# febrianrachmadi/dep-gan-im

Measured on AMD Instinct MI355X. Metric: 2D slices/sec (G+2D+GP train step), 256x256x1 fp32, higher is better.
Workload: dtype f32; 1 GPU; DEP-GAN-IM twoCritics canonical train step (critic-Y2 + critic-DEM + G update, WGAN-GP), batch 32 per GPU, 256x256x1; per_gpu_batch=32, global_batch=32, parallelism=dp1

## Files before the change

### dep_gan_im_amd/csrc/common.h

```cpp
#pragma once
#include <hip/hip_runtime.h>
#include <stdint.h>
#include <stddef.h>

typedef float f32x2 __attribute__((ext_vector_type(2)));
typedef float f32x4 __attribute__((ext_vector_type(4)));
typedef float f32x16 __attribute__((ext_vector_type(16)));

struct TView {
  float* p;
  long sB, sY, sX;
};

static inline TView make_view(float* p, int H, int W, int C) {
  TView v;
  v.p = p;
  v.sX = C;
  v.sY = (long)W * C;
  v.sB = (long)H * W * C;
  return v;
}
static inline TView make_view_slice(float* p, int H, int W, int Ctot, int c0) {
  TView v = make_view(p, H, W, Ctot);
  v.p = p + c0;
// ... 130 lines not shown
  static int cus[DG_MAX_DEVICES] = {};
  const int d = dg_device_slot();
  if (d >= 0 && cus[d]) return cus[d];
  int n = 256;
  hipDeviceProp_t p;
  if (d >= 0 && hipGetDeviceProperties(&p, d) == hipSuccess && p.multiProcessorCount > 0) n = p.multiProcessorCount;
  if (d >= 0) cus[d] = n;
  return n;
}

struct ConvPlan {
  int KS, Cin, Cout;
  int MF;
  int NT;
  int CK;
  int nNT, nCC;
  size_t packedFloats;
  int variant;
  int bf16;
};
ConvPlan dg_plan_conv(int KS, int Cin, int Cout);
ConvPlan dg_plan_conv_items(int KS, int Cin, int Cout, long items);
ConvPlan dg_plan_conv_bf16(int KS, int Cin, int Cout);
ConvPlan dg_plan_conv_split(int KS, int Cin, int Cout, int planes);
int dg_conv_igemm_bf16(const ConvPlan& pl, const ConvArgs& a, hipStream_t st);
static inline size_t dg_plan_elem_bytes(const ConvPlan& pl) { return pl.variant >= 200 ? 2 * (size_t)pl.bf16 : (pl.bf16 ? 2 : 4); }

struct PackJob {
  const float* src;
  float* dst;
  const float* kscale;
  int ntaps, srcI, srcO, io, transpose, flip;
  int NT, CK, nCC, Kdim, Ndim;
  int bf16;
  int tapg;
  int wino;
  unsigned total;
  unsigned per_nt;
  unsigned nt_stride;
  unsigned blk0, nblk;
};
int dg_pack_job(const ConvPlan& pl, const float* src, int srcI, int srcO, int io, int transpose, int flip,
                const float* kscale, float* dst, size_t nt_stride, PackJob* job);
unsigned dg_pack_layout(PackJob* jobs_host, int njobs);
int dg_pack_weights_batch(const PackJob* jobs_dev, int njobs, unsigned nblocks, hipStream_t st);

int dg_pack_weights(const ConvPlan& pl, const float* src, int srcI, int srcO, int io, int transpose, int flip,
                    const float* kscale, float* dst, hipStream_t st);

int dg_conv_igemm(const ConvPlan& pl, const ConvArgs& a, hipStream_t st);
int dg_conv_igemm_check(const ConvPlan& pl, const ConvArgs& a);
bool dg_conv_igemm_wp_supported(const ConvPlan& pl, const ConvArgs& a, bool force);
int dg_conv_igemm_wp(const ConvPlan& pl, const ConvArgs& a, hipStream_t st);
int dg_conv_igemm_tile(const ConvPlan& pl, const ConvArgs& a, hipStream_t st);
bool dg_conv_igemm_head_supported(const ConvPlan& pl, const ConvArgs& a);
ConvPlan dg_plan_conv_wino(int Cin, int Cout);
bool dg_conv_wino_supported(const ConvPlan& pl, const ConvArgs& a);
const char* dg_conv_wino_name(const ConvArgs& a);
int dg_conv_wino(const ConvPlan& pl, const ConvArgs& a, hipStream_t st);
void dg_conv_igemm_name(const ConvPlan& pl, const ConvArgs& a, char* buf, size_t cap);
int dg_conv_direct(int KS, const ConvArgs& a, hipStream_t st);

size_t dg_wgrad_part_floats(int KS, int B, int H, int W, int Cin, int Cout);
int dg_wgrad(int KS, const WgradArgs& a, int* nchunks, hipStream_t st);
int dg_wgrad_finish(const float* part, int nchunks, int ntaps, int Cin, int Cout, const float* scale, float* out,
                    float* raw, int accumulate, int oi, const float* colpart, int colC, const float* colscale,
                    float* colout, float* colraw, hipStream_t st);
int dg_wgrad_finish_rows(const float* part, int nchunks, int ntaps, int Cin, int Cout, const float* scale, float* out,
                         float* raw, int accumulate, int oi, const float* colpart, int colrows, int colC,
                         const float* colscale, float* colout, float* colraw, hipStream_t st);
int dg_wgrad_reduce(const float* part, int nchunks, int ntaps, int Cin, int Cout, const float* scale, float* out,
                    float* raw, int accumulate, int oi, hipStream_t st);

bool dg_wgrad_bf16_supported(int KS, int Cin, int Cout);
size_t dg_wgrad_bf16_part_floats(int KS, int B, int H, int W, int Cin, int Cout);
int dg_wgrad_bf16(int KS, const WgradArgs& a, int* nchunks, hipStream_t st);

size_t dg_wgrad_small_part_floats(int KS, int B, int H, int W, int Cin, int Cout);
int dg_wgrad_small(int KS, const WgradArgs& a, int* nchunks, hipStream_t st);
```

### dep_gan_im_amd/csrc/igemm_conv.hip

```cpp
#include <stdlib.h>

#include "common.h"
#include "epilogue.h"

__device__ __forceinline__ void store_packed(float* dst, size_t i, float v, int bf16) {
  if (bf16) reinterpret_cast<__bf16*>(dst)[i] = (__bf16)v;
  else dst[i] = v;
}
__device__ __forceinline__ void store_split(float* dst, size_t nt_base, int cc, int tap, int n, int k, float v, int planes,
                                            int tapg, int ntaps, int NT, int CK) {
  const int ng = ntaps / tapg, tg = tap / tapg, tl = tap - tg * tapg;
  __bf16* d = reinterpret_cast<__bf16*>(dst) + nt_base + ((size_t)cc * ng + tg) * (size_t)(planes * tapg * NT * CK);
  float rem = v;
  for (int p = 0; p < planes; ++p) {
    const __bf16 hb = (__bf16)rem;
    d[((size_t)p * tapg + tl) * (NT * CK) + (size_t)n * CK + k] = hb;
    rem -= (float)hb;
  }
}

template <int MF>
struct Mfma;
template <>
struct Mfma<32> {
// ... 388 lines not shown
      static DgOncePerDevice once_h;
      if (once_h.need()) {
        HIPCHECK(hipFuncSetAttribute(reinterpret_cast<const void*>(&igemm_conv_head_kernel<false>),
                                     hipFuncAttributeMaxDynamicSharedMemorySize, (int)lds));
        HIPCHECK(hipFuncSetAttribute(reinterpret_cast<const void*>(&igemm_conv_head_kernel<true>),
                                     hipFuncAttributeMaxDynamicSharedMemorySize, (int)lds));
      }
      if (G < total) hipLaunchKernelGGL((igemm_conv_head_kernel<true>), dim3((unsigned)G), dim3(256), lds, st, b);
      else hipLaunchKernelGGL((igemm_conv_head_kernel<false>), dim3((unsigned)G), dim3(256), lds, st, b);
      HIPCHECK(hipGetLastError());
      return DG_OK;
    }
  }
  static DgOncePerDevice once;
  if (once.need()) {
    HIPCHECK(hipFuncSetAttribute(reinterpret_cast<const void*>(&igemm_conv_kernel<MF, KS, CK, TAPG, false>),
                                 hipFuncAttributeMaxDynamicSharedMemorySize, (int)lds));
    HIPCHECK(hipFuncSetAttribute(reinterpret_cast<const void*>(&igemm_conv_kernel<MF, KS, CK, TAPG, true>),
                                 hipFuncAttributeMaxDynamicSharedMemorySize, (int)lds));
  }
  if (G < total)
    hipLaunchKernelGGL((igemm_conv_kernel<MF, KS, CK, TAPG, true>), dim3((unsigned)G), dim3(256), lds, st, b);
  else
    hipLaunchKernelGGL((igemm_conv_kernel<MF, KS, CK, TAPG, false>), dim3((unsigned)G), dim3(256), lds, st, b);
  HIPCHECK(hipGetLastError());
  return DG_OK;
}

static int dispatch_variant(const ConvPlan& pl, const ConvArgs& a, hipStream_t st, char* name_out, size_t name_cap) {
  switch (pl.variant) {
    case 0: return launch_variant<32, 3, 16, 9>(a, st, name_out, name_cap);
    case 1: return launch_variant<16, 3, 16, 9>(a, st, name_out, name_cap);
    case 2: return launch_variant<32, 5, 8, 25>(a, st, name_out, name_cap);
    case 3: return launch_variant<16, 5, 16, 25>(a, st, name_out, name_cap);
    case 4: return launch_variant<32, 1, 32, 1>(a, st, name_out, name_cap);
    case 5: return launch_variant<16, 1, 16, 1>(a, st, name_out, name_cap);
    case 8: return launch_variant<32, 3, 8, 9>(a, st, name_out, name_cap);
  }
  dg_set_error("dg_conv_igemm: bad variant %d", pl.variant);
  return DG_ERR_ARG;
}

bool dg_conv_igemm_head_supported(const ConvPlan& pl, const ConvArgs& a) {
  return (pl.variant == 8 || pl.variant == 9) && !pl.bf16 && a.Cout == 32 && a.groups <= 1 && a.ep.pool.p == nullptr && a.cpt <= 0 &&
         !a.ep.accumulate;
}

void dg_conv_igemm_name(const ConvPlan& pl, const ConvArgs& a, char* buf, size_t cap) {
  if (cap) buf[0] = 0;
  if (pl.variant < 0) { snprintf(buf, cap, "conv_direct"); return; }
  if (pl.bf16) { snprintf(buf, cap, pl.variant >= 200 ? "igemm_split_kernel" : "igemm_bf16_kernel"); return; }
  if (pl.variant == 9) { snprintf(buf, cap, "%s", dg_conv_wino_name(a)); return; }
  if (dg_conv_igemm_wp_supported(pl, a, false)) { snprintf(buf, cap, "igemm_wp_kernel<0>"); return; }
  dispatch_variant(pl, a, nullptr, buf, cap);
}

int dg_conv_igemm_check(const ConvPlan& pl, const ConvArgs& a) {
  if (pl.variant < 0) {
    dg_set_error("dg_conv_igemm: no MFMA variant for KS=%d Cin=%d Cout=%d", pl.KS, pl.Cin, pl.Cout);
    return DG_ERR_UNSUPPORTED;
  }
  auto misaligned = [](const TView& v) {
    return v.p && ((v.sX % 4) || (v.sY % 4) || (v.sB % 4) || (((uintptr_t)v.p) & 15));
  };
  if (misaligned(a.in) || misaligned(a.out) || misaligned(a.ep.res) || misaligned(a.ep.mask) ||
      misaligned(a.ep.out_pre) || (a.Cout % 4) || (a.ep.film_mul && (a.ep.film_ld % 4))) {
    dg_set_error("dg_conv_igemm: views must be 16-byte aligned (pointers, strides and Cout multiples of 4 floats)");
    return DG_ERR_ARG;
  }
  if (a.ep.pool.p && ((a.H | a.W) & 1 || misaligned(a.ep.pool) || a.groups > 1)) {
    dg_set_error("dg_conv_igemm: fused max-pool needs even H, W and a 16-byte aligned pooled view");
    return DG_ERR_ARG;
  }
  if (a.cpt > 0) {
    const int run = a.cpt * pl.CK;
    bool bad = a.groups > 1 || (a.Cin % run) != 0 || a.Cin / run > 4;
    for (int r = 0; !bad && r < a.Cin / run; ++r) bad = (a.in_run_off[r] % 4) != 0;
    if (bad) {
      dg_set_error("dg_conv_igemm: gathered K needs Cin = runs (<= 4) x cpt x %d channels and 16-byte run offsets", pl.CK);
      return DG_ERR_ARG;
    }
  }
  if (a.ep.head_out && !dg_conv_igemm_head_supported(pl, a)) {
    dg_set_error("dg_conv_igemm: the fused head needs the fp32 8-channel-chunk 3x3 kernel, 32 output channels, no pool");
    return DG_ERR_ARG;
  }
  return DG_OK;
}

static int conv_igemm_impl(const ConvPlan& pl, const ConvArgs& a_in, hipStream_t st, bool allow_wp) {
  ConvArgs a = a_in;
  const bool is_bf16 = pl.bf16 != 0;
  DGCHECK(dg_conv_igemm_check(pl, a));
  if (is_bf16) return dg_conv_igemm_bf16(pl, a, st);
  if (pl.variant == 9) return dg_conv_wino(pl, a, st);
  if (allow_wp && dg_conv_igemm_wp_supported(pl, a, false)) return dg_conv_igemm_wp(pl, a, st);
  return dispatch_variant(pl, a, st, nullptr, 0);
}

int dg_conv_igemm(const ConvPlan& pl, const ConvArgs& a, hipStream_t st) { return conv_igemm_impl(pl, a, st, true); }
int dg_conv_igemm_tile(const ConvPlan& pl, const ConvArgs& a, hipStream_t st) { return conv_igemm_impl(pl, a, st, false); }

__global__ void pack_weights_kernel(const float* __restrict__ src, float* __restrict__ dst, int ntaps, int srcI,
                                    int srcO, int io, int transpose, int flip, const float* __restrict__ kscale,
                                    int NT, int CK, int nCC, int Kdim, int Ndim, size_t total, int bf16, int tapg) {
  for (size_t i = blockIdx.x * (size_t)blockDim.x + threadIdx.x; i < total; i += (size_t)gridDim.x * blockDim.x) {
    size_t q = i;
    const int k = (int)(q % CK);
    q /= CK;
    const int n = (int)(q % NT);
    q /= NT;
    const int tap = (int)(q % ntaps);
    q /= ntaps;
    const int cc = (int)(q % nCC);
    const int nt = (int)(q / nCC);
    const int kk = cc * CK + k, nn = nt * NT + n;
    float v = 0.f;
    if (kk < Kdim && nn < Ndim) {
      const int ci = transpose ? nn : kk;
      const int co = transpose ? kk : nn;
      const int ts = flip ? (ntaps - 1 - tap) : tap;
      const size_t off = (size_t)ts * srcI * srcO + (io ? ((size_t)co * srcI + ci) : ((size_t)ci * srcO + co));
      v = src[off];
      if (kscale) v *= kscale[kk];
    }
    if (bf16 >= 2) store_split(dst, (size_t)nt * nCC * ntaps * NT * CK * bf16, cc, tap, n, k, v, bf16, tapg, ntaps, NT, CK);
    else store_packed(dst, i, v, bf16);
  }
}

__global__ __launch_bounds__(256) void pack_weights_batch_kernel(const PackJob* __restrict__ jobs, int njobs) {
  int lo = 0, hi = njobs - 1;
  while (lo < hi) {
    const int mid = (lo + hi + 1) >> 1;
    if (jobs[mid].blk0 <= blockIdx.x) lo = mid; else hi = mid - 1;
  }
  const PackJob J = jobs[lo];
  const unsigned b = blockIdx.x - J.blk0;
  if (J.wino) {
    const unsigned cols = J.total / 16u, plane = (unsigned)(J.NT * J.CK);
    for (unsigned i = b * 256u + threadIdx.x; i < cols; i += J.nblk * 256u) {
      unsigned q = i;
      const int k = (int)(q % J.CK);
      q /= J.CK;
      const int n = (int)(q % J.NT);
      q /= J.NT;
      const int cc = (int)(q % J.nCC);
      const int nt = (int)(q / J.nCC);
      const int kk = cc * J.CK + k, nn = nt * J.NT + n;
// ... 131 lines not shown
```

### dep_gan_im_amd/csrc/igemm_wp.hip

```cpp
#include <stdlib.h>

#include "common.h"
#include "epilogue.h"

namespace {

constexpr int WP_NW = 16;
constexpr int WP_TWX = 18, WP_TWY = 6;
constexpr int WP_PIX = WP_TWX * WP_TWY;
constexpr int WP_CK = 8, WP_CKP = 12;
constexpr int WP_WAVE_FLOATS = WP_PIX * WP_CKP;
constexpr int WP_SLOTS = WP_PIX * 2;
constexpr int WP_PIECES = (WP_SLOTS + 63) / 64;

template <int ABL>
__global__ __launch_bounds__(WP_NW * 64, 1) void igemm_wp_kernel(const ConvArgs a) {
  constexpr int MF = 32, NT = 32, MT = 2, KS = 3, TW = WP_TWX;
  typedef f32x16 acc_t;
  extern __shared__ __attribute__((aligned(16))) float smem[];
  const int tid = threadIdx.x;
  const int lane = tid & 63, wv = tid >> 6;
  const int r = lane & 31, h = lane >> 5;
  const int nCC = a.Cin / WP_CK;
  const int panelFloats = nCC * 9 * NT * WP_CK;
  float* panel = smem;
  float* wbuf = smem + panelFloats + wv * WP_WAVE_FLOATS;

  const unsigned nNT = (unsigned)a.lgy, nSup = (unsigned)a.lgx;
  const int supX = (a.W + 63) >> 6, supY = (a.H + 15) >> 4;
  unsigned id = blockIdx.x;
  auto decode = [&](unsigned i, int& st, int& nt) {
    if ((nSup & 7u) == 0) {
      const unsigned x = i & 7u, sl = i >> 3;
      nt = (int)(sl % nNT);
      st = (int)(x * (nSup >> 3) + sl / nNT);
    } else {
      st = (int)(i % nSup);
      nt = (int)(i / nSup);
    }
  };
  int st0, ntile;
  decode(id, st0, ntile);
  const int n0 = ntile * NT;

  {
    const float* src = a.w + (size_t)ntile * panelFloats;
    const int nq = panelFloats / 4;
    for (int q = tid; q < nq; q += WP_NW * 64) {
      const int row = q >> 1, half = q & 1;
      const f32x4 v = *reinterpret_cast<const f32x4*>(src + (size_t)q * 4);
      *reinterpret_cast<f32x4*>(panel + row * 8 + 4 * (half ^ ((row >> 2) & 1))) = v;
    }
  }
  __syncthreads();

  unsigned xgb[WP_PIECES], xlb[WP_PIECES];
  int xyx[WP_PIECES];
#pragma unroll
  for (int i = 0; i < WP_PIECES; ++i) {
    const int q = min(lane + 64 * i, WP_SLOTS - 1);
    const int pix = q >> 1, part = q & 1;
    const int ly = pix / TW, lx = pix - ly * TW;
    xgb[i] = 4u * (unsigned)(ly * (int)a.in.sY + lx * (int)a.in.sX + part * 4);
    xlb[i] = 4u * (unsigned)(pix * WP_CKP + part * 4);
    xyx[i] = (ly << 16) | (lx << 8) | (part * 4);
  }
  const bool in_last = lane < (WP_SLOTS - 64 * (WP_PIECES - 1));
  const unsigned wb0 = (unsigned)(size_t)(__attribute__((address_space(3))) float*)wbuf;
  int apix[MT];
#pragma unroll
  for (int mt = 0; mt < MT; ++mt) apix[mt] = ((2 * mt + (r >> 4)) * TW + (r & 15)) * WP_CKP + 4 * h;
  const int boff = r * 8 + 4 * (h ^ ((r >> 2) & 1));
  const int wrow = wv & 3, wcol = wv >> 2;

  for (;;) {
    int st, nt_unused;
    decode(id, st, nt_unused);
    const int sx = st % supX;
    int t = st / supX;
    const int sy = t % supY;
    const int b = t / supY;
    const int ty0 = sy * 16 + 4 * wrow, tx0 = sx * 64 + 16 * wcol;
    if (ty0 < a.H && tx0 < a.W) {
      const float* inb = a.in.p + (long)b * a.in.sB;
      const bool interior = ty0 >= 1 && ty0 + 5 <= a.H && tx0 >= 1 && tx0 + 17 <= a.W;
      const char* halo0 = reinterpret_cast<const char*>(inb + ((long)(ty0 - 1) * a.in.sY + (long)(tx0 - 1) * a.in.sX));
      f32x4 xr[WP_PIECES];
      auto prefetch = [&](int cc) {
        const char* src = halo0 + 4 * (long)cc * WP_CK;
        if (interior) {
#pragma unroll
          for (int i = 0; i < WP_PIECES - 1; ++i) xr[i] = *reinterpret_cast<const f32x4*>(src + xgb[i]);
          if (in_last) xr[WP_PIECES - 1] = *reinterpret_cast<const f32x4*>(src + xgb[WP_PIECES - 1]);
        } else {
#pragma unroll
          for (int i = 0; i < WP_PIECES; ++i) {
            const int iy = ty0 + (xyx[i] >> 16) - 1, ix = tx0 + ((xyx[i] >> 8) & 255) - 1;
            const bool ok = (i < WP_PIECES - 1 || in_last) && iy >= 0 && iy < a.H && ix >= 0 && ix < a.W;
            f32x4 v = {0.f, 0.f, 0.f, 0.f};
            if (ok) v = *reinterpret_cast<const f32x4*>(src + xgb[i]);
            xr[i] = v;
          }
        }
      };
      auto commit = [&]() {
#pragma unroll
        for (int i = 0; i < WP_PIECES - 1; ++i)
          *reinterpret_cast<__attribute__((address_space(3))) f32x4*>((size_t)(wb0 + xlb[i])) = xr[i];
        if (in_last)
          *reinterpret_cast<__attribute__((address_space(3))) f32x4*>((size_t)(wb0 + xlb[WP_PIECES - 1])) = xr[WP_PIECES - 1];
      };

      acc_t acc[MT];
#pragma unroll
      for (int mt = 0; mt < MT; ++mt)
#pragma unroll
        for (int j = 0; j < 16; ++j) acc[mt][j] = 0.f;

      prefetch(0);
      commit();
      for (int cc = 0; cc < nCC; ++cc) {
        if (!(ABL & 2) && cc + 1 < nCC) prefetch(cc + 1);
        const float* wp = panel + (size_t)cc * (9 * NT * WP_CK) + boff;
        f32x4 av[2][MT], bv[2];
        auto load_frag = [&](int tap, f32x4* a_, f32x4& b_) {
          const int ty = tap / KS, tx = tap - ty * KS;
          const int tapoff = (ty * TW + tx) * WP_CKP;
#pragma unroll
          for (int mt = 0; mt < MT; ++mt) a_[mt] = *reinterpret_cast<const f32x4*>(wbuf + apix[mt] + tapoff);
          b_ = *reinterpret_cast<const f32x4*>(wp + tap * (NT * WP_CK));
        };
        load_frag(0, av[0], bv[0]);
#pragma unroll
        for (int q = 0; q < 9; ++q) {
          if (q + 1 < 9) load_frag(q + 1, av[(q + 1) & 1], bv[(q + 1) & 1]);
          __builtin_amdgcn_sched_barrier(0);
#pragma unroll
          for (int j = 0; j < 4; ++j)
#pragma unroll
            for (int mt = 0; mt < MT; ++mt) {
              if (ABL & 4) acc[mt][j] += bv[q & 1][j] * av[q & 1][mt][j];
              else acc[mt] = __builtin_amdgcn_mfma_f32_32x32x2f32(bv[q & 1][j], av[q & 1][mt][j], acc[mt], 0, 0, 0);
            }
          __builtin_amdgcn_sched_barrier(0);
        }
        if (!(ABL & 2) && cc + 1 < nCC) commit();
      }

      const long out_goff = 0;
      if (ABL & 1) {
        if (acc[0][0] + acc[1][0] == 123.456f) a.out.p[0] = 1.f;
      } else {
#define EPI_PRE_SYNC ((void)0)
#define EPI_ES_BASE wbuf
#define EPI_PHASED
#define EPI_OYW ty0
#define EPI_FULL ((ty0 + 4 <= a.H) && (tx0 + 16 <= a.W))
#include "igemm_epilogue.inc"
#undef EPI_PRE_SYNC
#undef EPI_ES_BASE
#undef EPI_PHASED
#undef EPI_OYW
#undef EPI_FULL
      }
    }
    id += gridDim.x;
    if (id >= nSup * nNT) break;
  }
}

}

bool dg_conv_igemm_wp_supported(const ConvPlan& pl, const ConvArgs& a, bool force) {
  if (pl.variant != 8 || pl.bf16 || pl.KS != 3 || pl.CK != WP_CK) return false;
  if (a.Cin != pl.Cin || (a.Cin % WP_CK) || a.Cin > 64 || (a.Cout % 32) || a.groups > 1 || a.cpt > 0 || a.dbg) return false;
  if (a.ep.head_out) return false;
  const size_t lds = ((size_t)a.Cin * 9 * 32 + (size_t)WP_NW * WP_WAVE_FLOATS) * sizeof(float);
  if (lds > 160 * 1024) return false;
  if (force) return true;
  static int on = -1;
  if (on < 0) {
    const char* e = getenv("DEPGAN_IGEMM_WP");
    on = (e && atoi(e) != 0) ? 1 : 0;
  }
  if (!on) return false;
  const long sup = (long)a.B * cdiv(a.H, 16) * cdiv(a.W, 64);
  return (sup & 7) == 0 && sup * (a.Cout / 32) >= 256;
}

int dg_conv_igemm_wp(const ConvPlan& pl, const ConvArgs& a_in, hipStream_t st) {
  ConvArgs a = a_in;
  DGCHECK(dg_conv_igemm_check(pl, a));
  const size_t lds = ((size_t)a.Cin * 9 * 32 + (size_t)WP_NW * WP_WAVE_FLOATS) * sizeof(float);
  static DgOncePerDevice once;
  if (once.need())
    HIPCHECK(hipFuncSetAttribute(reinterpret_cast<const void*>(&igemm_wp_kernel<0>),
                                 hipFuncAttributeMaxDynamicSharedMemorySize, 160 * 1024));
  const int nNT = a.Cout / 32;
  a.lgx = a.B * cdiv(a.H, 16) * cdiv(a.W, 64);
  a.lgy = nNT;
  const long total = (long)a.lgx * nNT;
  long G = dg_cu_count();
  G -= G % (8L * nNT);
  if (G < 8L * nNT) G = 8L * nNT;
  if (G > total || (a.lgx & 7) != 0) G = total;
#ifdef DEPGAN_WP_ABLATIONS
  static int abl = -1;
  if (abl < 0) {
    const char* e = getenv("DEPGAN_WP_ABL");
    abl = e ? atoi(e) : 0;
  }
  if (abl) {
    static DgOncePerDevice once2;
    if (once2.need()) {
      HIPCHECK(hipFuncSetAttribute(reinterpret_cast<const void*>(&igemm_wp_kernel<1>), hipFuncAttributeMaxDynamicSharedMemorySize, 160 * 1024));
      HIPCHECK(hipFuncSetAttribute(reinterpret_cast<const void*>(&igemm_wp_kernel<2>), hipFuncAttributeMaxDynamicSharedMemorySize, 160 * 1024));
      HIPCHECK(hipFuncSetAttribute(reinterpret_cast<const void*>(&igemm_wp_kernel<3>), hipFuncAttributeMaxDynamicSharedMemorySize, 160 * 1024));
      HIPCHECK(hipFuncSetAttribute(reinterpret_cast<const void*>(&igemm_wp_kernel<4>), hipFuncAttributeMaxDynamicSharedMemorySize, 160 * 1024));
    }
    switch (abl) {
      case 1: hipLaunchKernelGGL((igemm_wp_kernel<1>), dim3((unsigned)G), dim3(WP_NW * 64), lds, st, a); break;
      case 2: hipLaunchKernelGGL((igemm_wp_kernel<2>), dim3((unsigned)G), dim3(WP_NW * 64), lds, st, a); break;
      case 3: hipLaunchKernelGGL((igemm_wp_kernel<3>), dim3((unsigned)G), dim3(WP_NW * 64), lds, st, a); break;
      default: hipLaunchKernelGGL((igemm_wp_kernel<4>), dim3((unsigned)G), dim3(WP_NW * 64), lds, st, a); break;
    }
    HIPCHECK(hipGetLastError());
    return DG_OK;
  }
#endif
  hipLaunchKernelGGL((igemm_wp_kernel<0>), dim3((unsigned)G), dim3(WP_NW * 64), lds, st, a);
  HIPCHECK(hipGetLastError());
  return DG_OK;
}
```

### dep_gan_im_amd/csrc/model.hip

```cpp
#include "model.h"
#include "train_ops.h"

#include <dlfcn.h>
#include <math.h>
#include <stdlib.h>
#include <stdarg.h>
#include <stdio.h>
#include <string.h>

static thread_local char g_err[1024] = "";
void dg_set_error(const char* fmt, ...) {
  va_list ap;
  va_start(ap, fmt);
  vsnprintf(g_err, sizeof(g_err), fmt, ap);
  va_end(ap);
}
const char* dg_get_error() { return g_err; }

void Net::add(const std::string& name, std::vector<int> shape, bool trainable) {
  PInfo pi;
  pi.name = name;
  pi.ndim = (int)shape.size();
  pi.size = 1;
  for (int i = 0; i < 4; ++i) {
// ... 1675 lines not shown
      N = B; C = L.Cout;
      break;
    }
  } else if (starts("d/act/") || starts("d/mixed/")) {
    const bool mixed = starts("d/mixed/");
    const std::string ln = mixed ? rest("d/mixed/") : rest("d/act/");
    for (size_t l = 0; l < c->dl.size(); ++l) {
      if (c->dl[l].name != ln) continue;
      if (mixed) {
        if (!c->dbg_mixed_valid || !c->dbg_mixed[l]) { dg_set_error("debug_tensor: %s was not captured (depgan_debug_capture)", name); return DG_ERR_ARG; }
        v = make_view(c->dbg_mixed[l], c->dl[l].H, c->dl[l].W, c->dl[l].Cout);
        N = B;
      } else {
        v = c->d_act[l].view();
        N = c->NB3;
      }
      H = c->dl[l].H; W = c->dl[l].W; C = c->dl[l].Cout;
      break;
    }
  }
  if (!v.p || N == 0) { dg_set_error("debug_tensor: unknown tensor '%s'", name); return DG_ERR_ARG; }
  shape[0] = N; shape[1] = H; shape[2] = W; shape[3] = C;
  if (!host) return DG_OK;
  const long need = (long)N * H * W * C;
  if (cap < need) { dg_set_error("debug_tensor: %s needs %ld floats, the buffer holds %ld", name, need, cap); return DG_ERR_ARG; }
  if (v.sY != (long)W * v.sX || v.sB != (long)H * v.sY) { dg_set_error("debug_tensor: %s is not a channel slice of a dense tensor", name); return DG_ERR_UNSUPPORTED; }
  HIPCHECK(hipStreamSynchronize(c->st));
  if (v.sX == C) {
    HIPCHECK(hipMemcpy(host, v.p, (size_t)need * sizeof(float), hipMemcpyDeviceToHost));
    return DG_OK;
  }
  float* tmp = nullptr;
  HIPCHECK(hipMalloc((void**)&tmp, (size_t)need * sizeof(float)));
  hipError_t e = hipMemcpy2D(tmp, (size_t)C * sizeof(float), v.p, (size_t)v.sX * sizeof(float), (size_t)C * sizeof(float),
                             (size_t)N * H * W, hipMemcpyDeviceToDevice);
  if (e == hipSuccess) e = hipMemcpy(host, tmp, (size_t)need * sizeof(float), hipMemcpyDeviceToHost);
  hipFree(tmp);
  if (e != hipSuccess) { dg_set_error("debug_tensor: copy of %s failed: %s", name, hipGetErrorString(e)); return DG_ERR_HIP; }
  return DG_OK;
}

static int op_conv_run(ConvArgs a, const float* w_hwio, int Cin, int Cout, int KS, int path, int bwd, hipStream_t st) {
  const int ci = a.Cin, co = a.Cout;
  ConvPlan pl = (path == 3) ? dg_plan_conv_bf16(KS, ci, co)
                : (path == 4 || path == 5) ? dg_plan_conv_split(KS, ci, co, path == 5 ? 3 : 2)
                : (path == 6) ? dg_plan_conv_items(KS, ci, co, 1L << 30) : dg_plan_conv(KS, ci, co);
  if (path == 7) pl = dg_plan_conv_items(KS, ci, co, 1L << 30);
  if (path == 8) {
    pl = (KS == 3) ? dg_plan_conv_wino(ci, co) : pl;
    if (pl.variant != 9 || !dg_conv_wino_supported(pl, a)) { dg_set_error("op_conv: the Winograd kernel does not cover this shape"); return DG_ERR_UNSUPPORTED; }
  }
  if ((path == 6 || path == 7) && pl.CK != 8) { dg_set_error("op_conv: the 8-channel-chunk variant does not cover this shape"); return DG_ERR_UNSUPPORTED; }
  if (path >= 3 && path <= 5 && !pl.bf16) { dg_set_error("op_conv: the bf16 MFMA kernel does not cover this shape"); return DG_ERR_UNSUPPORTED; }
  if (path == 1 && pl.variant < 0) { dg_set_error("op_conv: MFMA path not available for this shape"); return DG_ERR_UNSUPPORTED; }
  if (path != 2 && pl.variant >= 0) {
    float* wp = nullptr;
    HIPCHECK(hipMalloc((void**)&wp, pl.packedFloats * sizeof(float)));
    int rc = dg_pack_weights(pl, w_hwio, Cin, Cout, 0, bwd, bwd, nullptr, wp, st);
    if (rc == DG_OK) {
      a.w = wp;
      if (path == 7) {
        if (dg_conv_igemm_wp_supported(pl, a, true)) rc = dg_conv_igemm_wp(pl, a, st);
        else { dg_set_error("op_conv: the wave-private kernel does not cover this shape"); rc = DG_ERR_UNSUPPORTED; }
      } else if (path == 6) {
        rc = dg_conv_igemm_tile(pl, a, st);
      } else {
        rc = dg_conv_igemm(pl, a, st);
      }
    }
    hipStreamSynchronize(st);
    hipFree(wp);
    return rc;
  }
  a.w = w_hwio;
  if (!bwd) {
    a.wsT = (long)Cin * Cout; a.wsI = Cout; a.wsO = 1; a.flip = 0;
  } else {
    a.wsT = (long)Cin * Cout; a.wsI = 1; a.wsO = Cout; a.flip = 1;
  }
  return dg_conv_direct(KS, a, st);
}

static int op_conv(const float* in, const float* w_hwio, const float* bias, float* out, int B, int H, int W, int Cin,
                   int Cout, int KS, int relu, int path, int bwd, hipStream_t st) {
  const int ci = bwd ? Cout : Cin, co = bwd ? Cin : Cout;
  ConvArgs a;
  memset(&a, 0, sizeof(a));
  zero_ep(&a.ep);
  a.in = make_view(const_cast<float*>(in), H, W, ci);
  a.out = make_view(out, H, W, co);
  a.B = B; a.H = H; a.W = W; a.Cin = ci; a.Cout = co;
  a.ep.bias = bias;
  a.ep.relu = relu;
  return op_conv_run(a, w_hwio, Cin, Cout, KS, path, bwd, st);
}

int depgan_op_conv2d_stamps(const float* in, const float* w_hwio, float* out, int B, int H, int W, int Cin, int Cout,
                            int KS, unsigned long long* stamps, int reps, void* stream) {
  hipStream_t st = (hipStream_t)stream;
  ConvArgs a;
  memset(&a, 0, sizeof(a));
  zero_ep(&a.ep);
  a.in = make_view(const_cast<float*>(in), H, W, Cin);
  a.out = make_view(out, H, W, Cout);
  a.B = B; a.H = H; a.W = W; a.Cin = Cin; a.Cout = Cout;
  a.ep.relu = 1;
  ConvPlan pl = dg_plan_conv(KS, Cin, Cout);
  if (pl.variant < 0) { dg_set_error("no MFMA variant"); return DG_ERR_UNSUPPORTED; }
  float* wp = nullptr;
  HIPCHECK(hipMalloc((void**)&wp, pl.packedFloats * sizeof(float)));
  int rc = dg_pack_weights(pl, w_hwio, Cin, Cout, 0, 0, 0, nullptr, wp, st);
  a.w = wp;
  for (int i = 0; i < reps && rc == DG_OK; ++i) {
    a.dbg = (i == reps - 1) ? stamps : nullptr;
    rc = dg_conv_igemm(pl, a, st);
  }
  hipStreamSynchronize(st);
// ... 117 lines not shown
                       double thr, long long out_host[DEPGAN_EVAL_NCOUNT], void* stream) {
  if (!x || !pred || !out_host || nicg < 1 || npix < 0) { dg_set_error("eval_counts: bad argument"); return DG_ERR_ARG; }
  hipStream_t st = (hipStream_t)stream;
  unsigned long long* dev = nullptr;
  HIPCHECK(hipMalloc((void**)&dev, DEPGAN_EVAL_NCOUNT * sizeof(unsigned long long)));
  int rc = dg_eval_counts(x, nicg, pred, code_real, mask1, wmh1, mask2, wmh2, prob2, (size_t)npix, thr, dev, st);
  if (rc == DG_OK) {
    unsigned long long h[DEPGAN_EVAL_NCOUNT];
    if (hipMemcpyAsync(h, dev, sizeof(h), hipMemcpyDeviceToHost, st) != hipSuccess ||
        hipStreamSynchronize(st) != hipSuccess) {
      dg_set_error("eval_counts: copy back failed");
      rc = DG_ERR_HIP;
    } else {
      for (int k = 0; k < DEPGAN_EVAL_NCOUNT; ++k) out_host[k] = (long long)h[k];
    }
  }
  hipFree(dev);
  return rc;
}


static int op_alloc(float** p, size_t floats, const char* who) {
  if (hipMalloc((void**)p, (floats ? floats : 1) * sizeof(float)) != hipSuccess) {
    dg_set_error("%s: out of device memory (%zu floats)", who, floats);
    return DG_ERR_HIP;
  }
  return DG_OK;
}
static size_t op_scratch(long scratch_floats, size_t need) { return scratch_floats > 0 ? (size_t)scratch_floats : need; }

static bool op_view_bad(const float* p, long sB, long sY, long sX) { return !p || sB < 1 || sY < 1 || sX < 1; }

int depgan_op_conv2d_fused(const float* in, long isB, long isY, long isX, const float* w_hwio, const float* bias,
                           const float* scale, const float* shift, const float* film_mul, const float* film_add,
                           int film_ld, float* out, long osB, long osY, long osX, float* out_pre, long psB, long psY,
                           long psX, const float* res, long rsB, long rsY, long rsX, const float* mask, long msB,
                           long msY, long msX, float* pool, long qsB, long qsY, long qsX, const float* head_w,
                           const float* head_b, float* head_out, int head_tanh, int head_skip_out, int B, int H, int W,
                           int Cin, int Cout, int KS, int relu, int accumulate, int path, int bwd, void* stream) {
  if (op_view_bad(in, isB, isY, isX) || op_view_bad(out, osB, osY, osX) || !w_hwio || B < 1 || H < 1 || W < 1 || Cin < 1 ||
      Cout < 1 || (KS != 1 && KS != 3 && KS != 5) || (out_pre && op_view_bad(out_pre, psB, psY, psX)) ||
      (res && op_view_bad(res, rsB, rsY, rsX)) || (mask && op_view_bad(mask, msB, msY, msX)) ||
      (pool && op_view_bad(pool, qsB, qsY, qsX))) {
    dg_set_error("op_conv2d_fused: null or non-positive argument");
    return DG_ERR_ARG;
  }
  const int co = bwd ? Cin : Cout;
  if (!scale != !shift || !film_mul != !film_add || (film_mul && film_ld < co)) {
    dg_set_error("op_conv2d_fused: scale / shift and film_mul / film_add come in pairs, film_ld >= output channels");
    return DG_ERR_ARG;
  }
  if ((head_w || head_b || head_out) && !(head_w && head_b && head_out)) { dg_set_error("op_conv2d_fused: null head argument"); return DG_ERR_ARG; }
  if (head_skip_out && !head_out) { dg_set_error("op_conv2d_fused: head_skip_out without a head"); return DG_ERR_ARG; }
  if (path < 1 || path > 8) { dg_set_error("op_conv2d_fused: path must be 1 ... 8"); return DG_ERR_ARG; }
  ConvArgs a;
  memset(&a, 0, sizeof(a));
  zero_ep(&a.ep);
  a.in = op_view(in, isB, isY, isX);
  a.out = op_view(out, osB, osY, osX);
  a.B = B; a.H = H; a.W = W; a.Cin = bwd ? Cout : Cin; a.Cout = co;
  Epilogue& e = a.ep;
  e.bias = bias; e.scale = scale; e.shift = shift;
  e.film_mul = film_mul; e.film_add = film_add; e.film_ld = film_ld;
  e.out_pre = op_view_or_null(out_pre, psB, psY, psX);
  e.res = op_view_or_null(res, rsB, rsY, rsX);
  e.mask = op_view_or_null(mask, msB, msY, msX);
  e.pool = op_view_or_null(pool, qsB, qsY, qsX);
  e.relu = relu; e.accumulate = accumulate;
  e.head_w = head_w; e.head_b = head_b; e.head_out = head_out;
  e.head_tanh = head_tanh; e.head_skip_out = head_skip_out;
  return op_conv_run(a, w_hwio, Cin, Cout, KS, path, bwd ? 1 : 0, (hipStream_t)stream);
}

static int op_pack_jobs(PackJob* jobs, int n, hipStream_t st) {
  const unsigned nb = dg_pack_layout(jobs, n);
  PackJob* jd = nullptr;
  HIPCHECK(hipMalloc((void**)&jd, n * sizeof(PackJob)));
  hipError_t e = hipMemcpyAsync(jd, jobs, n * sizeof(PackJob), hipMemcpyHostToDevice, st);
  int rc = DG_OK;
  if (e != hipSuccess) { dg_set_error("op_pack_jobs: upload failed: %s", hipGetErrorString(e)); rc = DG_ERR_HIP; }
  if (rc == DG_OK) rc = dg_pack_weights_batch(jd, n, nb, st);
  hipStreamSynchronize(st);
  hipFree(jd);
  return rc;
}

int depgan_op_deconv2x2_igemm(int form, const float* in, long isB, long isY, long isX, const float* w_hwoi,
                              const float* bias, const float* scale, const float* shift, float* out, long osB, long osY,
                              long osX, const float* mask, long msB, long msY, long msX, int B, int H, int W, int Cin,
                              int Cout, int relu, int path, void* stream) {
  if (op_view_bad(in, isB, isY, isX) || op_view_bad(out, osB, osY, osX) || !w_hwoi || B < 1 || H < 1 || W < 1 || Cin < 1 ||
      Cout < 1 || (mask && op_view_bad(mask, msB, msY, msX))) {
    dg_set_error("op_deconv2x2_igemm: null or non-positive argument");
    return DG_ERR_ARG;
  }
  if (form < 0 || form > 2 || !scale != !shift || (path != 1 && path != 3 && path != 8)) {
    dg_set_error("op_deconv2x2_igemm: form must be 0, 1 or 2, path 1, 3 or 8, scale and shift come as a pair");
    return DG_ERR_ARG;
  }
  if (form == 0 ? mask != nullptr : (bias || scale || relu)) {
    dg_set_error("op_deconv2x2_igemm: the forward takes bias / scale / shift / relu, the backward-data forms a mask");
    return DG_ERR_ARG;
  }
  if (path == 8) { dg_set_error("op_deconv2x2_igemm: the Winograd kernel has no 1x1 form"); return DG_ERR_UNSUPPORTED; }
  auto plan = [&](int ci, int co) { return path == 3 ? dg_plan_conv_bf16(1, ci, co) : dg_plan_conv(1, ci, co); };
  auto covered = [&](const ConvPlan& p) { return p.variant >= 0 && (path == 3) == (p.bf16 != 0); };
  hipStream_t st = (hipStream_t)stream;
// ... 482 lines not shown
```

Before: 638.2 slices/s.

## Add weight-stationary wave-private MFMA kernel for 5x5 convolutions

Generalizes the wave-private 3x3 implicit-GEMM kernel into a template over MFMA size, kernel size and channel chunk, and instantiates a 5x5 variant where the whole weight panel stays resident in LDS while each wave walks 16x4 output tiles from a persistent grid. The default dispatch uses it for 5x5 convs with Cout equal to the MFMA width and Cin of 16 or 32 when there are enough work items. Halo loads switch to buffer loads with a readfirstlane'd resource, and a swizzled halo layout is added for CK=16. The cost is more LDS per block, one block per CU, and a heuristic gate that may pick it for shapes where the old tiled kernel was better.

```diff
diff --git a/dep_gan_im_amd/csrc/common.h b/dep_gan_im_amd/csrc/common.h
--- a/dep_gan_im_amd/csrc/common.h
+++ b/dep_gan_im_amd/csrc/common.h
@@ -206,6 +206,9 @@
 int dg_conv_igemm_check(const ConvPlan& pl, const ConvArgs& a);
 bool dg_conv_igemm_wp_supported(const ConvPlan& pl, const ConvArgs& a, bool force);
 int dg_conv_igemm_wp(const ConvPlan& pl, const ConvArgs& a, hipStream_t st);
+bool dg_conv_igemm_ws5_supported(const ConvPlan& pl, const ConvArgs& a, bool force);
+int dg_conv_igemm_ws5(const ConvPlan& pl, const ConvArgs& a, hipStream_t st);
+const char* dg_conv_igemm_ws5_name(const ConvPlan& pl);
 int dg_conv_igemm_tile(const ConvPlan& pl, const ConvArgs& a, hipStream_t st);
 bool dg_conv_igemm_head_supported(const ConvPlan& pl, const ConvArgs& a);
 ConvPlan dg_plan_conv_wino(int Cin, int Cout);
diff --git a/dep_gan_im_amd/csrc/igemm_conv.hip b/dep_gan_im_amd/csrc/igemm_conv.hip
--- a/dep_gan_im_amd/csrc/igemm_conv.hip
+++ b/dep_gan_im_amd/csrc/igemm_conv.hip
@@ -464,6 +464,7 @@
   if (pl.bf16) { snprintf(buf, cap, pl.variant >= 200 ? "igemm_split_kernel" : "igemm_bf16_kernel"); return; }
   if (pl.variant == 9) { snprintf(buf, cap, "%s", dg_conv_wino_name(a)); return; }
   if (dg_conv_igemm_wp_supported(pl, a, false)) { snprintf(buf, cap, "igemm_wp_kernel<0>"); return; }
+  if (dg_conv_igemm_ws5_supported(pl, a, false)) { snprintf(buf, cap, "%s", dg_conv_igemm_ws5_name(pl)); return; }
   dispatch_variant(pl, a, nullptr, buf, cap);
 }
 
@@ -507,6 +508,7 @@
   if (is_bf16) return dg_conv_igemm_bf16(pl, a, st);
   if (pl.variant == 9) return dg_conv_wino(pl, a, st);
   if (allow_wp && dg_conv_igemm_wp_supported(pl, a, false)) return dg_conv_igemm_wp(pl, a, st);
+  if (allow_wp && dg_conv_igemm_ws5_supported(pl, a, false)) return dg_conv_igemm_ws5(pl, a, st);
   return dispatch_variant(pl, a, st, nullptr, 0);
 }
 
diff --git a/dep_gan_im_amd/csrc/igemm_wp.hip b/dep_gan_im_amd/csrc/igemm_wp.hip
--- a/dep_gan_im_amd/csrc/igemm_wp.hip
+++ b/dep_gan_im_amd/csrc/igemm_wp.hip
@@ -6,28 +6,59 @@
 namespace {
 
 constexpr int WP_NW = 16;
-constexpr int WP_TWX = 18, WP_TWY = 6;
-constexpr int WP_PIX = WP_TWX * WP_TWY;
-constexpr int WP_CK = 8, WP_CKP = 12;
-constexpr int WP_WAVE_FLOATS = WP_PIX * WP_CKP;
-constexpr int WP_SLOTS = WP_PIX * 2;
-constexpr int WP_PIECES = (WP_SLOTS + 63) / 64;
-
-template <int ABL>
-__global__ __launch_bounds__(WP_NW * 64, 1) void igemm_wp_kernel(const ConvArgs a) {
-  constexpr int MF = 32, NT = 32, MT = 2, KS = 3, TW = WP_TWX;
+
+template <int MF, int KS, int CK>
+struct WpGeo {
+  static constexpr int NT = MF, MT = 64 / MF, PAD = KS / 2, NTAPS = KS * KS;
+  static constexpr int TWX = 16 + KS - 1, TWY = 4 + KS - 1;
+  static constexpr int PIX = TWX * TWY;
+  static constexpr int XV = CK / 4;
+  static constexpr int CKP = (KS == 3) ? CK + 4 : CK;
+  static constexpr int EPI_FLOATS = (MF == 32 ? 32 : 64) * (NT + 4);
+  static constexpr int WAVE_FLOATS = PIX * CKP > EPI_FLOATS ? PIX * CKP : EPI_FLOATS;
+  static constexpr int SLOTS = PIX * XV;
+  static constexpr int PIECES = (SLOTS + 63) / 64;
+  static __device__ __forceinline__ int panel_sw(int n) {
+    if (MF == 32) return (n >> (KS == 3 ? 2 : 4)) & 1;
+    return (0x78 >> (2 * (n >> 2))) & 3;
+  }
+  static __device__ __forceinline__ int halo_off(int pix, int part) {
+    if (CK == 16) return pix * CKP + 4 * (part ^ (((pix >> 2) & 1) << 1));
+    return pix * CKP + 4 * part;
+  }
+};
+
+template <int MF> struct WpMfma;
+template <> struct WpMfma<32> {
   typedef f32x16 acc_t;
+  static constexpr int NREG = 16;
+  static __device__ __forceinline__ acc_t run(float w, float x, acc_t c) { return __builtin_amdgcn_mfma_f32_32x32x2f32(w, x, c, 0, 0, 0); }
+};
+template <> struct WpMfma<16> {
+  typedef f32x4 acc_t;
+  static constexpr int NREG = 4;
+  static __device__ __forceinline__ acc_t run(float w, float x, acc_t c) { return __builtin_amdgcn_mfma_f32_16x16x4f32(w, x, c, 0, 0, 0); }
+};
+
+template <int MF, int KS, int CK, int ABL>
+static __device__ __forceinline__ void igemm_wp_body(const ConvArgs& a) {
+  typedef WpGeo<MF, KS, CK> G;
+  constexpr int NT = G::NT, MT = G::MT, TW = G::TWX, PAD = G::PAD, NTAPS = G::NTAPS, CKP = G::CKP;
+  constexpr int PIECES = G::PIECES, SLOTS = G::SLOTS, XV = G::XV;
+  typedef typename WpMfma<MF>::acc_t acc_t;
   extern __shared__ __attribute__((aligned(16))) float smem[];
   const int tid = threadIdx.x;
   const int lane = tid & 63, wv = tid >> 6;
-  const int r = lane & 31, h = lane >> 5;
-  const int nCC = a.Cin / WP_CK;
-  const int panelFloats = nCC * 9 * NT * WP_CK;
+  const int NW = (int)(blockDim.x >> 6);
+  const int r = lane % MF, h = lane / MF;
+  const int nCC = a.Cin / CK;
+  const int panelFloats = nCC * NTAPS * NT * CK;
   float* panel = smem;
-  float* wbuf = smem + panelFloats + wv * WP_WAVE_FLOATS;
+  float* wbuf = smem + panelFloats + wv * G::WAVE_FLOATS;
 
   const unsigned nNT = (unsigned)a.lgy, nSup = (unsigned)a.lgx;
-  const int supX = (a.W + 63) >> 6, supY = (a.H + 15) >> 4;
+  const int bxN = (a.W + 15) >> 4, bandsY = (a.H + 15) >> 4;
+  const int nItems = a.B * bandsY * bxN * 4;
   unsigned id = blockIdx.x;
   auto decode = [&](unsigned i, int& st, int& nt) {
     if ((nSup & 7u) == 0) {
@@ -41,106 +72,131 @@
   };
   int st0, ntile;
   decode(id, st0, ntile);
-  const int n0 = ntile * NT;
 
   {
     const float* src = a.w + (size_t)ntile * panelFloats;
     const int nq = panelFloats / 4;
-    for (int q = tid; q < nq; q += WP_NW * 64) {
-      const int row = q >> 1, half = q & 1;
+    for (int q = tid; q < nq; q += (int)blockDim.x) {
+      const int row = q / XV, part = q % XV;
       const f32x4 v = *reinterpret_cast<const f32x4*>(src + (size_t)q * 4);
-      *reinterpret_cast<f32x4*>(panel + row * 8 + 4 * (half ^ ((row >> 2) & 1))) = v;
+      *reinterpret_cast<f32x4*>(panel + row * CK + 4 * (part ^ G::panel_sw(row % NT))) = v;
     }
   }
   __syncthreads();
 
-  unsigned xgb[WP_PIECES], xlb[WP_PIECES];
-  int xyx[WP_PIECES];
-#pragma unroll
-  for (int i = 0; i < WP_PIECES; ++i) {
-    const int q = min(lane + 64 * i, WP_SLOTS - 1);
-    const int pix = q >> 1, part = q & 1;
+  unsigned xgb[PIECES];
+  constexpr int PSTEP = 64 / XV;
+  static_assert(PSTEP % 8 == 0, "the halo swizzle must repeat from piece to piece");
+  const int xpart = lane % XV, xpix0 = lane / XV;
+#pragma unroll
+  for (int i = 0; i < PIECES; ++i) {
+    const int pix = min(xpix0 + PSTEP * i, G::PIX - 1);
     const int ly = pix / TW, lx = pix - ly * TW;
-    xgb[i] = 4u * (unsigned)(ly * (int)a.in.sY + lx * (int)a.in.sX + part * 4);
-    xlb[i] = 4u * (unsigned)(pix * WP_CKP + part * 4);
-    xyx[i] = (ly << 16) | (lx << 8) | (part * 4);
-  }
-  const bool in_last = lane < (WP_SLOTS - 64 * (WP_PIECES - 1));
+    xgb[i] = 4u * (unsigned)(ly * (int)a.in.sY + lx * (int)a.in.sX + xpart * 4);
+  }
+  const unsigned xlb0 = 4u * (unsigned)G::halo_off(xpix0, xpart);
+  const bool in_last = lane < (SLOTS - 64 * (PIECES - 1));
   const unsigned wb0 = (unsigned)(size_t)(__attribute__((address_space(3))) float*)wbuf;
   int apix[MT];
 #pragma unroll
-  for (int mt = 0; mt < MT; ++mt) apix[mt] = ((2 * mt + (r >> 4)) * TW + (r & 15)) * WP_CKP + 4 * h;
-  const int boff = r * 8 + 4 * (h ^ ((r >> 2) & 1));
-  const int wrow = wv & 3, wcol = wv >> 2;
+  for (int mt = 0; mt < MT; ++mt)
+    apix[mt] = (MF == 32) ? ((2 * mt + (r >> 4)) * TW + (r & 15)) * CKP + 4 * h : (mt * TW + r) * CKP + 4 * h;
+  int asw[KS][2];
+#pragma unroll
+  for (int tx = 0; tx < KS; ++tx)
+#pragma unroll
+    for (int par = 0; par < 2; ++par)
+      asw[tx][par] = (CK == 16) ? (r + tx) * CKP + 4 * (h ^ (((((r + tx) >> 2) & 1) ^ par) << 1)) : 0;
+  const int boff = r * CK + 4 * (h ^ G::panel_sw(r));
 
   for (;;) {
     int st, nt_unused;
     decode(id, st, nt_unused);
-    const int sx = st % supX;
-    int t = st / supX;
-    const int sy = t % supY;
-    const int b = t / supY;
-    const int ty0 = sy * 16 + 4 * wrow, tx0 = sx * 64 + 16 * wcol;
-    if (ty0 < a.H && tx0 < a.W) {
+    const int item = st * NW + wv;
+    const int wrow = item & 3;
+    int t = item >> 2;
+    const int bxi = t % bxN;
+    t /= bxN;
+    const int sy = t % bandsY;
+    const int b = t / bandsY;
+    const int ty0 = sy * 16 + 4 * wrow, tx0 = bxi * 16;
+    if (item < nItems && ty0 < a.H) {
+      int n0 = ntile * NT;
+      asm volatile("" : "+s"(n0));
       const float* inb = a.in.p + (long)b * a.in.sB;
-      const bool interior = ty0 >= 1 && ty0 + 5 <= a.H && tx0 >= 1 && tx0 + 17 <= a.W;
-      const char* halo0 = reinterpret_cast<const char*>(inb + ((long)(ty0 - 1) * a.in.sY + (long)(tx0 - 1) * a.in.sX));
-      f32x4 xr[WP_PIECES];
+      const bool interior = ty0 >= PAD && ty0 + 4 + PAD <= a.H && tx0 >= PAD && tx0 + 16 + PAD <= a.W;
+      const char* halo0 = reinterpret_cast<const char*>(inb + ((long)(ty0 - PAD) * a.in.sY + (long)(tx0 - PAD) * a.in.sX));
+      const unsigned long long hu = (unsigned long long)halo0;
+      const unsigned hlo = __builtin_amdgcn_readfirstlane((unsigned)hu), hhi = __builtin_amdgcn_readfirstlane((unsigned)(hu >> 32));
+      const __amdgpu_buffer_rsrc_t halo_rsrc =
+          __builtin_amdgcn_make_buffer_rsrc((void*)(((unsigned long long)hhi << 32) | hlo), 0, 0x7FFFFFFF, 0x00020000);
+      f32x4 xr[PIECES];
       auto prefetch = [&](int cc) {
-        const char* src = halo0 + 4 * (long)cc * WP_CK;
+        const char* src = halo0 + 4 * (long)cc * CK;
         if (interior) {
-#pragma unroll
-          for (int i = 0; i < WP_PIECES - 1; ++i) xr[i] = *reinterpret_cast<const f32x4*>(src + xgb[i]);
-          if (in_last) xr[WP_PIECES - 1] = *reinterpret_cast<const f32x4*>(src + xgb[WP_PIECES - 1]);
+          typedef int i32x4 __attribute__((ext_vector_type(4)));
+#pragma unroll
+          for (int i = 0; i < PIECES - 1; ++i)
+            xr[i] = __builtin_bit_cast(f32x4, __builtin_amdgcn_raw_buffer_load_b128(halo_rsrc, (int)xgb[i], 4 * cc * CK, 0));
+          if (in_last)
+            xr[PIECES - 1] =
+                __builtin_bit_cast(f32x4, __builtin_amdgcn_raw_buffer_load_b128(halo_rsrc, (int)xgb[PIECES - 1], 4 * cc * CK, 0));
         } else {
-#pragma unroll
-          for (int i = 0; i < WP_PIECES; ++i) {
-            const int iy = ty0 + (xyx[i] >> 16) - 1, ix = tx0 + ((xyx[i] >> 8) & 255) - 1;
-            const bool ok = (i < WP_PIECES - 1 || in_last) && iy >= 0 && iy < a.H && ix >= 0 && ix < a.W;
+          int xp = xpix0;
+          asm volatile("" : "+v"(xp));
+#pragma unroll
+          for (int i = 0; i < PIECES; ++i) {
+            const int pix = min(xp + PSTEP * i, G::PIX - 1);
+            const int ly = pix / TW, lx = pix - ly * TW;
+            const int iy = ty0 + ly - PAD, ix = tx0 + lx - PAD;
+            const bool ok = (i < PIECES - 1 || in_last) && iy >= 0 && iy < a.H && ix >= 0 && ix < a.W;
             f32x4 v = {0.f, 0.f, 0.f, 0.f};
-            if (ok) v = *reinterpret_cast<const f32x4*>(src + xgb[i]);
+            if (ok) v = *reinterpret_cast<const f32x4*>(src + 4 * (ly * (int)a.in.sY + lx * (int)a.in.sX + xpart * 4));
             xr[i] = v;
           }
         }
       };
       auto commit = [&]() {
 #pragma unroll
-        for (int i = 0; i < WP_PIECES - 1; ++i)
-          *reinterpret_cast<__attribute__((address_space(3))) f32x4*>((size_t)(wb0 + xlb[i])) = xr[i];
+        for (int i = 0; i < PIECES - 1; ++i)
+          *reinterpret_cast<__attribute__((address_space(3))) f32x4*>((size_t)(wb0 + xlb0 + 4u * PSTEP * CKP * i)) = xr[i];
         if (in_last)
-          *reinterpret_cast<__attribute__((address_space(3))) f32x4*>((size_t)(wb0 + xlb[WP_PIECES - 1])) = xr[WP_PIECES - 1];
+          *reinterpret_cast<__attribute__((address_space(3))) f32x4*>((size_t)(wb0 + xlb0 + 4u * PSTEP * CKP * (PIECES - 1))) =
+              xr[PIECES - 1];
       };
 
       acc_t acc[MT];
 #pragma unroll
       for (int mt = 0; mt < MT; ++mt)
 #pragma unroll
-        for (int j = 0; j < 16; ++j) acc[mt][j] = 0.f;
+        for (int j = 0; j < WpMfma<MF>::NREG; ++j) acc[mt][j] = 0.f;
 
       prefetch(0);
       commit();
       for (int cc = 0; cc < nCC; ++cc) {
         if (!(ABL & 2) && cc + 1 < nCC) prefetch(cc + 1);
-        const float* wp = panel + (size_t)cc * (9 * NT * WP_CK) + boff;
+        const float* wp = panel + (size_t)cc * (NTAPS * NT * CK) + boff;
         f32x4 av[2][MT], bv[2];
         auto load_frag = [&](int tap, f32x4* a_, f32x4& b_) {
           const int ty = tap / KS, tx = tap - ty * KS;
-          const int tapoff = (ty * TW + tx) * WP_CKP;
-#pragma unroll
-          for (int mt = 0; mt < MT; ++mt) a_[mt] = *reinterpret_cast<const f32x4*>(wbuf + apix[mt] + tapoff);
-          b_ = *reinterpret_cast<const f32x4*>(wp + tap * (NT * WP_CK));
+#pragma unroll
+          for (int mt = 0; mt < MT; ++mt) {
+            if (CK == 16) a_[mt] = *reinterpret_cast<const f32x4*>(wbuf + asw[tx][(mt + ty) & 1] + (mt + ty) * TW * CKP);
+            else a_[mt] = *reinterpret_cast<const f32x4*>(wbuf + apix[mt] + (ty * TW + tx) * CKP);
+          }
+          b_ = *reinterpret_cast<const f32x4*>(wp + tap * (NT * CK));
         };
         load_frag(0, av[0], bv[0]);
 #pragma unroll
-        for (int q = 0; q < 9; ++q) {
-          if (q + 1 < 9) load_frag(q + 1, av[(q + 1) & 1], bv[(q + 1) & 1]);
+        for (int q = 0; q < NTAPS; ++q) {
+          if (q + 1 < NTAPS) load_frag(q + 1, av[(q + 1) & 1], bv[(q + 1) & 1]);
           __builtin_amdgcn_sched_barrier(0);
 #pragma unroll
           for (int j = 0; j < 4; ++j)
 #pragma unroll
             for (int mt = 0; mt < MT; ++mt) {
               if (ABL & 4) acc[mt][j] += bv[q & 1][j] * av[q & 1][mt][j];
-              else acc[mt] = __builtin_amdgcn_mfma_f32_32x32x2f32(bv[q & 1][j], av[q & 1][mt][j], acc[mt], 0, 0, 0);
+              else acc[mt] = WpMfma<MF>::run(bv[q & 1][j], av[q & 1][mt][j], acc[mt]);
             }
           __builtin_amdgcn_sched_barrier(0);
         }
@@ -153,13 +209,17 @@
       } else {
 #define EPI_PRE_SYNC ((void)0)
 #define EPI_ES_BASE wbuf
-#define EPI_PHASED
 #define EPI_OYW ty0
 #define EPI_FULL ((ty0 + 4 <= a.H) && (tx0 + 16 <= a.W))
+        if constexpr (MF == 32) {
+#define EPI_PHASED
 #include "igemm_epilogue.inc"
+#undef EPI_PHASED
+        } else {
+#include "igemm_epilogue.inc"
+        }
 #undef EPI_PRE_SYNC
 #undef EPI_ES_BASE
-#undef EPI_PHASED
 #undef EPI_OYW
 #undef EPI_FULL
       }
@@ -169,13 +229,27 @@
   }
 }
 
-}
+template <int ABL>
+__global__ __launch_bounds__(WP_NW * 64, 1) void igemm_wp_kernel(const ConvArgs a) {
+  igemm_wp_body<32, 3, 8, ABL>(a);
+}
+
+constexpr int ws5_nwmax(int MF) { return MF == 32 ? 16 : 12; }
+template <int MF, int CK>
+__global__ __launch_bounds__(ws5_nwmax(MF) * 64, 1) void igemm_ws5_kernel(const ConvArgs a) {
+  igemm_wp_body<MF, 5, CK, 0>(a);
+}
+
+}
+
+typedef WpGeo<32, 3, 8> Wp3;
+static long wp_groups(const ConvArgs& a, int nw) { return cdiv((long)a.B * cdiv(a.H, 16) * cdiv(a.W, 16) * 4, nw); }
 
 bool dg_conv_igemm_wp_supported(const ConvPlan& pl, const ConvArgs& a, bool force) {
-  if (pl.variant != 8 || pl.bf16 || pl.KS != 3 || pl.CK != WP_CK) return false;
-  if (a.Cin != pl.Cin || (a.Cin % WP_CK) || a.Cin > 64 || (a.Cout % 32) || a.groups > 1 || a.cpt > 0 || a.dbg) return false;
+  if (pl.variant != 8 || pl.bf16 || pl.KS != 3 || pl.CK != 8) return false;
+  if (a.Cin != pl.Cin || (a.Cin % 8) || a.Cin > 64 || (a.Cout % 32) || a.groups > 1 || a.cpt > 0 || a.dbg) return false;
   if (a.ep.head_out) return false;
-  const size_t lds = ((size_t)a.Cin * 9 * 32 + (size_t)WP_NW * WP_WAVE_FLOATS) * sizeof(float);
+  const size_t lds = ((size_t)a.Cin * 9 * 32 + (size_t)WP_NW * Wp3::WAVE_FLOATS) * sizeof(float);
   if (lds > 160 * 1024) return false;
   if (force) return true;
   static int on = -1;
@@ -184,20 +258,20 @@
     on = (e && atoi(e) != 0) ? 1 : 0;
   }
   if (!on) return false;
-  const long sup = (long)a.B * cdiv(a.H, 16) * cdiv(a.W, 64);
+  const long sup = wp_groups(a, WP_NW);
   return (sup & 7) == 0 && sup * (a.Cout / 32) >= 256;
 }
 
 int dg_conv_igemm_wp(const ConvPlan& pl, const ConvArgs& a_in, hipStream_t st) {
   ConvArgs a = a_in;
   DGCHECK(dg_conv_igemm_check(pl, a));
-  const size_t lds = ((size_t)a.Cin * 9 * 32 + (size_t)WP_NW * WP_WAVE_FLOATS) * sizeof(float);
+  const size_t lds = ((size_t)a.Cin * 9 * 32 + (size_t)WP_NW * Wp3::WAVE_FLOATS) * sizeof(float);
   static DgOncePerDevice once;
   if (once.need())
     HIPCHECK(hipFuncSetAttribute(reinterpret_cast<const void*>(&igemm_wp_kernel<0>),
                                  hipFuncAttributeMaxDynamicSharedMemorySize, 160 * 1024));
   const int nNT = a.Cout / 32;
-  a.lgx = a.B * cdiv(a.H, 16) * cdiv(a.W, 64);
+  a.lgx = (int)wp_groups(a, WP_NW);
   a.lgy = nNT;
   const long total = (long)a.lgx * nNT;
   long G = dg_cu_count();
@@ -232,3 +306,64 @@
   HIPCHECK(hipGetLastError());
   return DG_OK;
 }
+
+template <int MF, int CK>
+static int ws5_waves(int Cin) {
+  const long panel = (long)Cin * 25 * MF, wave = WpGeo<MF, 5, CK>::WAVE_FLOATS;
+  long nw = (160L * 1024 / 4 - panel) / wave;
+  static int cap = -1;
+  if (cap < 0) {
+    const char* e = getenv("DEPGAN_IGEMM_WS5_WAVES");
+    cap = (e && atoi(e) >= 4) ? atoi(e) : 16;
+  }
+  if (nw > cap) nw = cap;
+  return (int)(nw < ws5_nwmax(MF) ? nw : ws5_nwmax(MF));
+}
+static int ws5_waves_of(const ConvPlan& pl, int Cin) { return pl.MF == 32 ? ws5_waves<32, 8>(Cin) : ws5_waves<16, 16>(Cin); }
+
+bool dg_conv_igemm_ws5_supported(const ConvPlan& pl, const ConvArgs& a, bool force) {
+  if ((pl.variant != 2 && pl.variant != 3) || pl.bf16 || pl.KS != 5) return false;
+  if (pl.CK != (pl.MF == 32 ? 8 : 16)) return false;
+  if (a.Cin != pl.Cin || a.Cout != pl.Cout || a.Cout != pl.MF || (a.Cin != 16 && a.Cin != 32)) return false;
+  if (a.groups > 1 || a.cpt > 0 || a.dbg || a.ep.head_out) return false;
+  if (force) return true;
+  static int mode = -2;
+  if (mode == -2) {
+    const char* e = getenv("DEPGAN_IGEMM_WS5");
+    mode = e ? (atoi(e) != 0 ? 1 : 0) : -1;
+  }
+  if (mode == 0) return false;
+  const long items = (long)a.B * cdiv(a.H, 4) * cdiv(a.W, 16);
+  const long slots = (long)dg_cu_count() * ws5_waves_of(pl, a.Cin);
+  if (items < 2 * slots) return false;
+  if (mode == 1) return true;
+  if (a.Cin == 32 && a.Cout == 16) return false;
+  if (a.Cin == 32 && a.Cout == 32) return items >= 4 * slots;
+  return true;
+}
+
+const char* dg_conv_igemm_ws5_name(const ConvPlan& pl) { return pl.MF == 32 ? "igemm_ws5_kernel<32,8>" : "igemm_ws5_kernel<16,16>"; }
+
+template <int MF, int CK>
+static int ws5_launch(ConvArgs& a, hipStream_t st) {
+  const int nw = ws5_waves<MF, CK>(a.Cin);
+  const size_t lds = ((size_t)a.Cin * 25 * MF + (size_t)nw * WpGeo<MF, 5, CK>::WAVE_FLOATS) * sizeof(float);
+  static DgOncePerDevice once;
+  if (once.need())
+    HIPCHECK(hipFuncSetAttribute(reinterpret_cast<const void*>(&igemm_ws5_kernel<MF, CK>),
+                                 hipFuncAttributeMaxDynamicSharedMemorySize, 160 * 1024));
+  a.lgx = (int)wp_groups(a, nw);
+  a.lgy = 1;
+  long G = dg_cu_count();
+  if ((a.lgx & 7) == 0) G -= G % 8;
+  if (G > a.lgx || G < 1) G = a.lgx;
+  hipLaunchKernelGGL((igemm_ws5_kernel<MF, CK>), dim3((unsigned)G), dim3(nw * 64), lds, st, a);
+  HIPCHECK(hipGetLastError());
+  return DG_OK;
+}
+
+int dg_conv_igemm_ws5(const ConvPlan& pl, const ConvArgs& a_in, hipStream_t st) {
+  ConvArgs a = a_in;
+  DGCHECK(dg_conv_igemm_check(pl, a));
+  return pl.MF == 32 ? ws5_launch<32, 8>(a, st) : ws5_launch<16, 16>(a, st);
+}
diff --git a/dep_gan_im_amd/csrc/model.hip b/dep_gan_im_amd/csrc/model.hip
--- a/dep_gan_im_amd/csrc/model.hip
+++ b/dep_gan_im_amd/csrc/model.hip
@@ -1751,6 +1751,8 @@
   }
   if ((path == 6 || path == 7) && pl.CK != 8) { dg_set_error("op_conv: the 8-channel-chunk variant does not cover this shape"); return DG_ERR_UNSUPPORTED; }
   if (path >= 3 && path <= 5 && !pl.bf16) { dg_set_error("op_conv: the bf16 MFMA kernel does not cover this shape"); return DG_ERR_UNSUPPORTED; }
+  if (path == 9 && KS != 5) { dg_set_error("op_conv: path 9 is the weight-stationary 5x5 kernel, KS must be 5"); return DG_ERR_ARG; }
+  if (path == 9 && !dg_conv_igemm_ws5_supported(pl, a, true)) { dg_set_error("op_conv: the weight-stationary 5x5 kernel does not cover this shape"); return DG_ERR_UNSUPPORTED; }
   if (path == 1 && pl.variant < 0) { dg_set_error("op_conv: MFMA path not available for this shape"); return DG_ERR_UNSUPPORTED; }
   if (path != 2 && pl.variant >= 0) {
     float* wp = nullptr;
@@ -1761,7 +1763,9 @@
       if (path == 7) {
         if (dg_conv_igemm_wp_supported(pl, a, true)) rc = dg_conv_igemm_wp(pl, a, st);
         else { dg_set_error("op_conv: the wave-private kernel does not cover this shape"); rc = DG_ERR_UNSUPPORTED; }
-      } else if (path == 6) {
+      } else if (path == 9) {
+        rc = dg_conv_igemm_ws5(pl, a, st);
+      } else if (path == 6 || path == 1) {
         rc = dg_conv_igemm_tile(pl, a, st);
       } else {
         rc = dg_conv_igemm(pl, a, st);
@@ -1985,7 +1989,7 @@
   }
   if ((head_w || head_b || head_out) && !(head_w && head_b && head_out)) { dg_set_error("op_conv2d_fused: null head argument"); return DG_ERR_ARG; }
   if (head_skip_out && !head_out) { dg_set_error("op_conv2d_fused: head_skip_out without a head"); return DG_ERR_ARG; }
-  if (path < 1 || path > 8) { dg_set_error("op_conv2d_fused: path must be 1 ... 8"); return DG_ERR_ARG; }
+  if (path < 1 || path > 9) { dg_set_error("op_conv2d_fused: path must be 1 ... 9"); return DG_ERR_ARG; }
   ConvArgs a;
   memset(&a, 0, sizeof(a));
   zero_ep(&a.ep);
```

Result: faster. 648.6 slices/s (median of 6 runs) (+1.6%).
